# cgbur/llama2.zig

Hardware: AMD Instinct MI355X
Metric: tokens/s (argmax, -t 0) (higher is better)
Workload: dtype f32; 1 GPU; llama2-7b shape, fp32 llama2.c-v0 checkpoint (dim 4096, hidden 11008, L 32, H 32, kv 32, V 32000, S 2048), greedy from BOS, seeded synthetic weights; parallelism=1 GPU

## Files before the change

### llama2.zig_amd/csrc/forward.cpp

```cpp
#include <algorithm>
#include <cmath>
#include <cstdlib>
#include <cstring>
#include <mutex>

#include "batch_host.h"
#include "l2z_state.h"

namespace l2z {

struct Prof {
    std::vector<hipEvent_t> ev;
    std::vector<int> kind;
};

#define L2Z_LAUNCH(kind_id, expr)                                                         \
    do {                                                                                  \
        hipEvent_t _a = nullptr, _b = nullptr;                                            \
        if (prof) {                                                                       \
            L2Z_HIP(hipEventCreate(&_a));                                                 \
            L2Z_HIP(hipEventCreate(&_b));                                                 \
            L2Z_HIP(hipEventRecord(_a, st));                                              \
        }                                                                                 \
        L2Z_HIP(expr);                                                                    \
// ... 85 lines not shown
        L2Z_TRY(comm_allreduce(s->comm, s->part, s->x, dim, gi, was_pushed, st));
        if (prof != nullptr) {
            L2Z_HIP(hipEventRecord(eb, st));
            prof->ev.push_back(ea);
            prof->ev.push_back(eb);
            prof->kind.push_back(KIND_GATHER);
        }
        return L2Z_OK;
    };
    auto x_in = [&](MatvecArgs &a, const float *plain, int g, size_t count_per_rank) {
        a.x = plain;
        if (consume && g >= 1) a.xin = comm_ll_in(s->comm, g, count_per_rank);
    };
    auto push_to = [&](MatvecArgs &a, int which) {
        if (!can_push) return;
        a.push = s->d_push + which;
        a.push_ctl = ctl;
        a.push_gi = comm_gi(lc, gi + 1);
    };
    auto col_shard = [&](MatvecArgs &a, const float *wcols, const float *x_loc, int n_pad, int *epi) {
        a.w0 = wcols;
        a.x = x_loc;
        a.n = n_pad;
        a.rows0 = c.dim;
        a.out0 = s->part;
        a.resid = sh.rank == 0 ? s->x : nullptr;
        *epi = sh.rank == 0 ? EPI_RESID : EPI_STORE;
        push_to(a, 1);
    };
    const bool pk = s->packed_w && !sb && sh.world == 1 && !consume;
    const auto pk_slot = [&](int k, int l, int j = 0) -> const l2z_weights::PkMat * {
        return pk && ((s->packed_kinds >> k) & 1) ? w->pk_slot(k, l, j) : nullptr;
    };
    for (int l = 0; l < c.n_layers; l++) {
        float *kc = s->key_cache + (size_t)l * c.seq_len * sh.kvd_loc;
        float *vc = s->value_cache + (size_t)l * c.seq_len * sh.kvd_loc;
        const size_t kvh_stride = (size_t)c.seq_len * sh.hs;
        const bool fused = s->fused_qkv_attn && !split && only_stage < 0;
        if (fused && kind(KIND_QKV)) {
            FusedQkvAttnArgs a = {};
            a.wq = w->wq + (size_t)l * dim * dim;
            a.wk = w->wk + (size_t)l * dim * dim;
            a.wv = w->wv + (size_t)l * dim * dim;
            a.rms_w = w->rms_att + (size_t)l * dim; a.x = s->x; a.q_out = s->q;
            a.kcache = kc; a.vcache = vc; a.xb = s->xb; a.pos_ptr = s->d_pos; a.rope = s->rope;
            a.n = c.dim; a.head_size = sh.hs; a.seq_len = c.seq_len; a.kv_dim = sh.kvd_loc;
            a.kv_row = sh.hs; a.kv_head = kvh_stride;
            L2Z_LAUNCH(KIND_QKV, launch_fused_qkv_attn(a, c.n_heads, st));
        }
        if (!fused && want() && kind(KIND_QKV)) {
            MatvecArgs a = {};
            a.w0 = w->wq + (size_t)l * sh.dim_loc * dim;
            a.w1 = w->wk + (size_t)l * sh.kvd_loc * dim;
            a.w2 = w->wv + (size_t)l * sh.kvd_loc * dim;
            a.out0 = s->q; a.out1 = kc; a.out2 = vc;
            a.rows0 = sh.dim_loc; a.rows1 = sh.kvd_loc; a.rows2 = sh.kvd_loc;
            a.pos_stride1 = sh.hs; a.pos_stride2 = sh.hs; a.kv_head_stride = kvh_stride;
            a.n = c.dim; a.rms_w = w->rms_att + (size_t)l * dim;
            x_in(a, s->x, gi, sh.dim_loc);
            a.pos_ptr = s->d_pos; a.rope = s->rope; a.head_size = sh.hs; a.rope_segs = 2;
            const auto *pq = pk_slot(KIND_QKV, l, 0), *pkk = pk_slot(KIND_QKV, l, 1), *pv = pk_slot(KIND_QKV, l, 2);
            if (pq && pkk && pv) {
                a.pk = pq->p; a.pk_e = pq->e;
                a.pk1 = pkk->p; a.pk_e1 = pkk->e;
                a.pk2 = pv->p; a.pk_e2 = pv->e;
            }
// ... 15 lines not shown
                L2Z_LAUNCH(KIND_ATTN, launch_attention_split(a, sh.heads_loc, s->attn_nch,
                                                             s->d_attn_part, s->d_attn_cnt, st, variant == ATTN_SPLIT_S));
            else
                L2Z_LAUNCH(KIND_ATTN, launch_attention(a, sh.heads_loc, st, variant == ATTN_SHORT ? 1 : 0));
        }
        if (!sb) L2Z_TRY(gather(s->xb, sh.dim_loc));
        if (want() && kind(KIND_WO)) {
            MatvecArgs a = {};
            int epi = EPI_RESID;
            if (sb) {
                col_shard(a, w->wo + (size_t)l * dim * sh.dimc_pad, s->xb + sh.dim0, sh.dimc_pad, &epi);
            } else {
                a.w0 = w->wo + (size_t)l * sh.dim_loc * dim;
                a.out0 = s->x + sh.dim0; a.resid = s->x + sh.dim0;
                a.rows0 = sh.dim_loc; a.n = c.dim;
                x_in(a, s->xb, gi, sh.dim_loc);
                push_to(a, 1);
                if (const auto *p = pk_slot(KIND_WO, l)) { a.pk = p->p; a.pk_e = p->e; }
            }
            L2Z_LAUNCH(KIND_WO, launch_matvec(a, PRO_NONE, epi, mb, g_cus, st, nullptr, &pushed));
        }
        if (sb) L2Z_TRY(reduce());
        else L2Z_TRY(gather(s->x, sh.dim_loc));
        if (want() && kind(KIND_FFN13)) {
            MatvecArgs a = {};
            a.w0 = w->w1 + (size_t)l * sh.hid_loc * 2 * dim;
            a.w1 = w->w3 + (size_t)l * sh.hid_loc * 2 * dim;
            a.out0 = sb ? s->hb : s->hb + sh.hid0;
            a.rows0 = sh.hid_loc; a.rows1 = sh.hid_loc; a.n = c.dim;
            a.rms_w = w->rms_ffn + (size_t)l * dim;
            x_in(a, s->x, gi, sh.dim_loc);
            if (!sb) push_to(a, 2);
            if (const auto *p = pk_slot(KIND_FFN13, l)) { a.pk = p->p; a.pk_e = p->e; }
            L2Z_LAUNCH(KIND_FFN13, launch_matvec(a, PRO_RMS, EPI_SWIGLU, mb, g_cus, st, nullptr, &pushed));
        }
        if (!sb) L2Z_TRY(gather(s->hb, sh.hid_loc));
        if (want() && kind(KIND_FFN2)) {
            MatvecArgs a = {};
            int epi = EPI_RESID;
            if (sb) {
                col_shard(a, w->w2 + (size_t)l * dim * sh.hidc_pad, s->hb, sh.hidc_pad, &epi);
            } else {
                a.w0 = w->w2 + (size_t)l * sh.dim_loc * hid;
                a.out0 = s->x + sh.dim0; a.resid = s->x + sh.dim0;
                a.rows0 = sh.dim_loc; a.n = c.hidden_dim;
                x_in(a, s->hb, gi, sh.hid_loc);
                push_to(a, 1);
                if (const auto *p = pk_slot(KIND_FFN2, l)) { a.pk = p->p; a.pk_e = p->e; }
            }
            L2Z_LAUNCH(KIND_FFN2, launch_matvec(a, PRO_NONE, epi, mb, g_cus, st, nullptr, &pushed));
        }
        if (sb) L2Z_TRY(reduce());
        else L2Z_TRY(gather(s->x, sh.dim_loc));
    }
    if (want() && kind(KIND_CLS)) {
        MatvecArgs a = {};
        a.w0 = w->wcls; a.out0 = s->logits + sh.v0;
        a.rows0 = sh.v_loc; a.n = c.dim; a.rms_w = w->rms_final;
        x_in(a, s->x, gi, sh.dim_loc);
        a.part_val = s->d_part_val; a.part_idx = s->d_part_idx; a.row_offset = sh.v0;
        const bool fuse = (sh.world == 1 || xchg || (only_kind >= 0 && with_step && s->comm && !s->comm->nccl && !s->comm->p2p)) &&
                          matvec_vector_width(c.dim);
        int grid = 0;
        if (!xchg) push_to(a, 3);
        if (const auto *p = fuse ? pk_slot(KIND_CLS, 0) : nullptr) { a.pk = p->p; a.pk_e = p->e; }
        L2Z_LAUNCH(KIND_CLS, launch_matvec(a, PRO_RMS, fuse ? EPI_ARGMAX : EPI_STORE, mb, g_cus, st,
// ... 443 lines not shown
```

### llama2.zig_amd/csrc/l2z_internal.h

```cpp
#pragma once

#include <hip/hip_runtime.h>

#include <cstdarg>
#include <cstdint>
#include <cstdio>
#include <string>
#include <vector>

#include "../../include/llama2_hip.h"
#include "../../include/llama2_hip_test.h"

namespace l2z {

struct P2pArgs;

struct LLIn {
    const unsigned long long *slots;
    unsigned slot_floats;
    unsigned count;
    int gi;
    int *ctl;
    int *h_err;
    long long timeout_ticks;
// ... 61 lines not shown
    const float *tok_emb;
    float *x;
    int dim;
    int advance;
    int *epoch_ctl;
    int epoch_add;
    const P2pArgs *xchg;
    int xchg_gi;
};

struct MatvecArgs {
    const float *w0, *w1, *w2;
    float *out0, *out1, *out2;
    int rows0, rows1, rows2;
    int pos_stride1, pos_stride2;
    size_t kv_head_stride;
    int n;
    const float *x;
    const float *rms_w;
    const float *resid;
    const int *pos_ptr;
    const float2 *rope;
    int head_size;
    int rope_segs;
    float *part_val;
    int *part_idx;
    int row_offset;
    const P2pArgs *push;
    const int *push_ctl;
    int push_gi;
    LLIn xin;
    const uint32_t *pk, *pk1, *pk2;
    int pk_e, pk_e1, pk_e2;
    int tl_slot;
};

struct AttnArgs {
    const float *q;
    const float *kcache;
    const float *vcache;
    float *xb;
    const int *pos_ptr;
    int head_size;
    int kv_row;
    size_t kv_head;
    int kv_mul;
    int seq_len;
    const P2pArgs *push;
    const int *push_ctl;
    int push_gi;
    int tl_seq;
};


struct FusedQkvAttnArgs {
    const float *wq, *wk, *wv;
    const float *rms_w, *x;
    float *q_out;
    float *kcache, *vcache;
    float *xb;
    const int *pos_ptr;
    const float2 *rope;
    int n;
    int head_size, seq_len, kv_dim;
    int kv_row;
    size_t kv_head;
// ... 188 lines not shown
```

### llama2.zig_amd/csrc/l2z_state.h

```cpp
#pragma once
#include <cstdint>
#include <vector>

#include "kv_pages.h"
#include "l2z_comm.h"
#include "l2z_internal.h"
#include "tunables.h"

namespace l2z {

struct BatchScratch;
struct WideScratch;

struct Shard {
    int rank = 0, world = 1;
    int hs = 0;
    int dim0 = 0, dim_loc = 0;
    int kvd_loc = 0;
    int heads_loc = 0;
    int hid0 = 0, hid_loc = 0;
    int v0 = 0, v_loc = 0;
    bool scheme_b = false;
    int dimc_pad = 0, hidc_pad = 0;
};
int pad_cols(int n);
int make_shard(const l2z_config &c, const l2z_comm *comm, Shard *out);

enum ShardKind { REPL, BY_Q_HEADS, BY_KV_HEADS, BY_HIDDEN, BY_DIM_ROWS, BY_VOCAB, SKIP };

struct TensorDesc {
    const char *name;
    size_t offset;
    size_t layers, rows, cols;
    ShardKind kind;
    float scale, bias;
    size_t count() const { return layers * rows * cols; }
};
std::vector<TensorDesc> tensor_table(const l2z_config &c, bool shared);
void shard_rows(const TensorDesc &d, const Shard &s, size_t *r0, size_t *r1);
// ... 81 lines not shown
    void *sc_ws = nullptr, *sc_seq = nullptr;
    size_t sc_ws_bytes = 0;
    int sc_cap = 0, sc_slab_n = 0;
    int sc_slab_force = 0;
    float *d_probs = nullptr;
    float *h_stage = nullptr;
    float *d_smp_ctl = nullptr, *h_smp_ctl = nullptr, *d_smp_scratch = nullptr;
    float *d_part_val = nullptr;
    int *d_part_idx = nullptr;
    int n_part = 0;
    int n_part_step = 0, n_part_fwd = 0;
    float *d_attn_part = nullptr;
    int *d_attn_cnt = nullptr;
    int attn_nch = 0;
    int attn_split_pos = 0;
    int attn_short_pos = 0;
    int attn_split_wide_pos = 0;
    uint64_t graph_w_uid = 0;
    hipGraphExec_t g_forward[4] = {nullptr, nullptr, nullptr, nullptr}, g_step[4] = {nullptr, nullptr, nullptr, nullptr};
    hipGraphExec_t g_sample[4] = {nullptr, nullptr, nullptr, nullptr};
    bool use_graphs = true;
    int host_pos = 0;
    bool done = false;
    std::vector<int32_t> h_prompt;
    l2z::P2pArgs *d_push = nullptr;
    int n_gathers = 0;
    bool ll_consume = false;
    bool xchg_steps = false;
    bool logits_partial = false;
    bool fused_qkv_attn = false;
    int max_blocks = 0;
    bool packed_w = true;
    int packed_kinds = -1;
    int tl_attn_seq = 0;
    l2z::BatchScratch *bt = nullptr;
    float *rg_k = nullptr, *rg_v = nullptr;
    void *rg_tab = nullptr;
    int rg_cap = 0;
    l2z::WideScratch *wd = nullptr;
};

namespace l2z {

struct Prof;
int check_pair(const l2z_config *config, const l2z_runstate *s, const l2z_weights *w, bool paged_ok = false);
enum { ATTN_SHORT = 0, ATTN_HEAD = 1, ATTN_SPLIT_S = 2, ATTN_SPLIT = 3, ATTN_VARIANTS = 4 };
enum StepKind { STEP_NONE = 0, STEP_GREEDY = 1, STEP_SAMPLE = 2 };
int enqueue_forward(l2z_runstate *s, const l2z_weights *w, StepKind step, Prof *prof, int only_stage,
                    int variant, int only_kind = -1);
int attn_variant(const l2z_runstate *s, int pos);
int run_forward(l2z_runstate *s, const l2z_weights *w, StepKind step, int pos);
int ensure_logits(l2z_runstate *s);
void drop_graphs(l2z_runstate *s);

constexpr int kPrefillMinPrompt = L2Z_PREFILL_MIN_PROMPT;
bool prefill_enabled();
bool prefill_usable(const l2z_runstate *s);
bool prefill_shard_takes_the_unsharded_kernels(const l2z_config &c, const Shard &sh);
int prefill_check(const l2z_config *config, const l2z_runstate *s);
struct ScoreCall;
int prefill_tokens(l2z_runstate *s, const l2z_weights *w, const int32_t *tokens, int n_tokens, int pos0,
                   const ScoreCall *score = nullptr);

int prefill_scratch(l2z_runstate *s, int need);
int prefill_ragged_chunk(l2z_runstate *s, const l2z_weights *w, const int32_t *tokens, int P, const RaggedChunk &rg);
int prefill_last_logits(l2z_runstate *s, const l2z_weights *w);
// ... 19 lines not shown
```

### llama2.zig_amd/csrc/matvec.hip

```cpp
#include <type_traits>

#include "argmax_rule.h"
#include "matvec_device.h"
#include "packed_w.h"

namespace l2z {
namespace {

__device__ __forceinline__ void dot2_scalar(const float *__restrict__ pa,
                                            const float *__restrict__ pb, const float *xs, int n,
                                            float &ra, float &rb)
{
    const int lane = threadIdx.x & 63;
    float sa = 0.0f, sb = 0.0f;
    for (int j = lane; j < n; j += kWave) {
        const float xv = xs[j];
        sa = fmaf(pa[j], xv, sa);
        sb = fmaf(pb[j], xv, sb);
    }
    ra = wave_sum(sa);
    rb = wave_sum(sb);
}

template <int LPR>
struct MvGeom {
    static constexpr int RW = kWave / LPR;
    static constexpr int U = (LPR == 64) ? 4 : 6;
};

template <int LPR>
__device__ __forceinline__ void mv_load(const float *pa, const float *pb, int c0, int n4,
                                        v4f (&wa)[MvGeom<LPR>::U], v4f (&wb)[MvGeom<LPR>::U])
{
    constexpr int U = MvGeom<LPR>::U;
    const v4f *a4 = (const v4f *)pa, *b4 = (const v4f *)pb;
#pragma unroll
    for (int k = 0; k < U; k++) {
// ... 219 lines not shown
    {
        const bool last = b + 1 == n_batches;
        const uint32_t *src = pp + (last ? last_off : (size_t)b * (4 * 64 * pk::kMaxLaneDw) + (size_t)wave_u * (64 * pk::kMaxLaneDw));
        s_in[P] = (XC == 4 || !last) ? 4 : s_last;
        e31[P] = e_pt;
        pk_load_raw(src, threadIdx.x & 63, XC == 4 ? 4 : s_in[P], raw[P]);
    }
    template <int P>
    __device__ __forceinline__ void deliver()
    {
        if constexpr (XC == 4) {
            pk_decode_lane<4>(raw[P], e31[P], wa, wb);
        } else {
            switch (s_in[P]) {
                case 4: pk_decode_lane<4>(raw[P], e31[P], wa, wb); break;
                case 3: pk_decode_lane<3>(raw[P], e31[P], wa, wb); break;
                case 2: pk_decode_lane<2>(raw[P], e31[P], wa, wb); break;
                case 1: pk_decode_lane<1>(raw[P], e31[P], wa, wb); break;
                default: pk_decode_lane<0>(raw[P], e31[P], wa, wb); break;
            }
        }
    }
};

#ifdef L2Z_TIMELINE
constexpr int kMtlSlots = 256, kMtlBlocks = 512;
__device__ long long g_mtl[kMtlSlots * kMtlBlocks * 8];
unsigned long long g_mtl_launches = 0;
#define L2Z_MTL(i) tl[i] = wall_clock64()
#else
#define L2Z_MTL(i) do { } while (0)
#endif

template <int PRO, int EPI, int XC, bool LL, bool PK = false>
__global__ __launch_bounds__(kBlock) void matvec_row_kernel(const MatvecArgs a)
{
    constexpr int U = kRowU;
    using Src = typename std::conditional<PK, RowPacked<EPI, XC>, RowF32<EPI, XC>>::type;
    constexpr int NS = Src::kSets;
    extern __shared__ __attribute__((aligned(16))) float lds[];
#ifdef L2Z_TIMELINE
    long long tl[8] = {0, 0, 0, 0, 0, 0, 0, 0};
#endif
    L2Z_MTL(0);
    MvLocals m_ = mv_locals<EPI>(a);
    if constexpr (PK) m_.push = nullptr;
    const MvLocals m = m_;
    const int n4 = m.n >> 2;
    const int n_batches = (n4 + kBlock * U - 1) / (kBlock * U);
    const int n4_pad = n_batches * (kBlock * U);
    float *xs = lds;
    float *scratch = lds + 4 * n4_pad;
    float *part = scratch + kScratch;
    const v4f *xs4 = (const v4f *)xs;
    const int tid = threadIdx.x, lane = tid & 63, wave = tid >> 6;
    const int n_units = m.n_pairs;
    const int ustride = gridDim.x;

    XStage<PRO, XC, LL> xst;
    xst.issue(a.x, a.xin, a.rms_w, n4);
    int u = blockIdx.x;
    Src src;
    src.init(m, n4, n_batches);
    src.point(m, u);
    EpiIn ein = epi_prefetch<EPI>(m, u, tid == 0);
    EpiIn ein_next = ein;
    src.template issue<0>(0);
    L2Z_MTL(1);
    xst.finish(a.x, a.rms_w, m.n, n4_pad, xs, scratch);
    L2Z_MTL(2);

    int iu = u, ib = 0;
    bool imore = true;
    auto advance = [&]() __attribute__((always_inline)) {
        const MvStep s = mv_step(iu, ib, n_batches, ustride, n_units);
        imore = s.more;
        if (s.more) {
            if (s.unit_done) src.point(m, s.u_next);
            iu = s.u_next;
            ib = s.b_next;
        }
    };
    advance();

    v4f acc_a = {0.f, 0.f, 0.f, 0.f}, acc_b = {0.f, 0.f, 0.f, 0.f};
    ArgmaxCand best;
    int b = 0, parity = 0;
    auto step = [&](auto set, auto ahead) __attribute__((always_inline)) -> bool {
        constexpr int P = decltype(set)::value;
        const MvStep s = mv_step(u, b, n_batches, ustride, n_units);
        auto prefetch_next = [&]() __attribute__((always_inline)) {
            if (s.more && s.unit_done) ein_next = epi_prefetch<EPI>(m, s.u_next, tid == 0);
        };
        if constexpr (NS > 1) {
            prefetch_next();
            if constexpr (decltype(ahead)::value) {
                if constexpr (EPI == EPI_SWIGLU) asm volatile("s_waitcnt vmcnt(0)" ::: "memory");
                src.template issue<(P + 1) % NS>(ib);
                advance();
            }
        }
        src.template deliver<P>();
#pragma unroll
        for (int k = 0; k < U; k++) {
            const v4f xv = xs4[b * (kBlock * U) + tid + kBlock * k];
            acc_a = fma4(src.wa[k], xv, acc_a);
            acc_b = fma4(src.wb[k], xv, acc_b);
        }
        if constexpr (NS == 1) {
            prefetch_next();
            if (imore) {
                src.template issue<0>(ib);
                advance();
            }
        }
#ifdef L2Z_TIMELINE
        tl[6]++;
#endif
        if (s.unit_done) {
            const float sa = wave_sum(hsum4(acc_a));
            const float sb = wave_sum(hsum4(acc_b));
            float *pp_ = part + parity * (2 * kWaves);
            if (lane == 0) {
                pp_[wave] = sa;
                pp_[kWaves + wave] = sb;
            }
            __syncthreads();
            if (tid == 0) {
                const float ta = ((pp_[0] + pp_[1]) + pp_[2]) + pp_[3];
                const float tb = ((pp_[kWaves] + pp_[kWaves + 1]) + pp_[kWaves + 2]) + pp_[kWaves + 3];
                pair_epilogue<EPI>(m, u, ta, tb, true, ein);
                if (EPI == EPI_ARGMAX) {
                    const int ra_ = 2 * u, rb_ = ra_ + 1;
                    argmax_take(best, ta, ra_ + a.row_offset);
                    if (rb_ < m.total_rows) argmax_take(best, tb, rb_ + a.row_offset);
                }
            }
            ein = ein_next;
            parity ^= 1;
            acc_a = v4f{0.f, 0.f, 0.f, 0.f};
            acc_b = v4f{0.f, 0.f, 0.f, 0.f};
#ifdef L2Z_TIMELINE
            if (tl[7]++ == 0) L2Z_MTL(3);
            L2Z_MTL(4);
#endif
        }
        u = s.u_next;
        b = s.b_next;
        return !s.more;
    };
    using Set0 = std::integral_constant<int, 0>;
    using Set1 = std::integral_constant<int, 1>;
    static_assert(NS == 1 || NS == 2, "register sets of a source");
    if constexpr (NS == 1) {
        while (!step(Set0{}, std::false_type{})) {}
    } else {
        while (true) {
            if (!imore) { step(Set0{}, std::false_type{}); break; }
            step(Set0{}, std::true_type{});
            if (!imore) { step(Set1{}, std::false_type{}); break; }
            step(Set1{}, std::true_type{});
        }
    }
    if (EPI == EPI_ARGMAX && tid == 0) {
        a.part_val[blockIdx.x] = best.v;
        a.part_idx[blockIdx.x] = best.i;
    }
#ifdef L2Z_TIMELINE
    L2Z_MTL(5);
    if (tid == 0 && (unsigned)a.tl_slot < (unsigned)kMtlSlots && blockIdx.x < kMtlBlocks) {
        long long *o = g_mtl + ((size_t)a.tl_slot * kMtlBlocks + blockIdx.x) * 8;
        for (int i = 0; i < 8; i++) o[i] = tl[i];
    }
#endif
}

template <int PRO, int EPI>
__global__ __launch_bounds__(kBlock) void matvec_scalar_kernel(const MatvecArgs a)
{
    extern __shared__ __attribute__((aligned(16))) float lds[];
    const MvLocals m = mv_locals<EPI>(a);
    float *xs = lds;
    float *scratch = lds + ((m.n + 3) & ~3);
    stage_x_scalar<PRO>(a.x, a.rms_w, m.n, xs, scratch);
    const int lane = threadIdx.x & 63, wave = threadIdx.x >> 6;
    for (int u = blockIdx.x * kWaves + wave; u < m.n_pairs; u += gridDim.x * kWaves) {
        const float *pa, *pb;
        pair_rows<EPI>(m, u, pa, pb);
        float sa, sb;
        dot2_scalar(pa, pb, xs, m.n, sa, sb);
        pair_epilogue<EPI>(m, u, sa, sb, lane == 0, epi_prefetch<EPI>(m, u, lane == 0));
    }
}

int lpr_for(int n4)
{
    int l = 8;
    while (l < 64 && l * 6 < n4) l <<= 1;
    return l;
}

struct MvLaunch {
    const void *fn;
    int lpr, u;
};

template <int PRO, int EPI, int LPR, int XC, bool LL>
MvLaunch mv_entry()
{
    return {reinterpret_cast<const void *>(&matvec_kernel<PRO, EPI, LPR, XC, LL>), LPR, MvGeom<LPR>::U};
}

template <int PRO, int EPI, bool LL>
MvLaunch mv_pick(int lpr, bool big_x)
{
    if (lpr == 8) return mv_entry<PRO, EPI, 8, 4, LL>();
    if (lpr == 16) return mv_entry<PRO, EPI, 16, 4, LL>();
    if (lpr == 32) return mv_entry<PRO, EPI, 32, 4, LL>();
    return big_x ? mv_entry<PRO, EPI, 64, 12, LL>() : mv_entry<PRO, EPI, 64, 4, LL>();
}

template <int PRO, int EPI, bool LL, bool PK = false>
const void *mv_row_fn(bool big_x)
{
    return big_x ? reinterpret_cast<const void *>(&matvec_row_kernel<PRO, EPI, 12, LL, PK>)
                 : reinterpret_cast<const void *>(&matvec_row_kernel<PRO, EPI, 4, LL, PK>);
}

#define L2Z_MV_COMBOS(X)                     \
    X(PRO_NONE, EPI_STORE,  0, 1, 0)         \
    X(PRO_NONE, EPI_RESID,  1, 1, 1)         \
    X(PRO_RMS,  EPI_STORE,  1, 1, 0)         \
    X(PRO_RMS,  EPI_ROPE,   1, 1, 1)         \
    X(PRO_RMS,  EPI_SWIGLU, 1, 1, 1)         \
    X(PRO_RMS,  EPI_ARGMAX, 1, 0, 1)
#define L2Z_IF_1(...) __VA_ARGS__
#define L2Z_IF_0(...)

const void *mv_row_pick_packed(int pro, int epi, bool big_x)
{
#define X(P, E, LL, SC, PK) L2Z_IF_##PK(if (pro == P && epi == E) return mv_row_fn<P, E, false, true>(big_x);)
    L2Z_MV_COMBOS(X)
#undef X
    return nullptr;
}

const void *mv_row_pick(int pro, int epi, bool big_x, bool ll)
{
#define X(P, E, LL, SC, PK)                                           \
    if (pro == P && epi == E && !ll) return mv_row_fn<P, E, false>(big_x); \
    L2Z_IF_##LL(if (pro == P && epi == E && ll) return mv_row_fn<P, E, true>(big_x);)
    L2Z_MV_COMBOS(X)
#undef X
    return nullptr;
}

MvLaunch mv_pick_pe(int pro, int epi, int lpr, bool big_x, bool vec, bool ll)
{
#define X(P, E, LL, SC, PK)                                                                \
    if (pro == P && epi == E && vec && !ll) return mv_pick<P, E, false>(lpr, big_x);       \
    L2Z_IF_##LL(if (pro == P && epi == E && vec && ll) return mv_pick<P, E, true>(lpr, big_x);) \
    L2Z_IF_##SC(if (pro == P && epi == E && !vec && !ll)                                   \
                    return MvLaunch{reinterpret_cast<const void *>(&matvec_scalar_kernel<P, E>), 0, 0};)
    L2Z_MV_COMBOS(X)
#undef X
    return {nullptr, 0, 0};
}
#undef L2Z_MV_COMBOS
#undef L2Z_IF_1
#undef L2Z_IF_0

__global__ __launch_bounds__(256) void stream_read_kernel(const v4f *__restrict__ p, size_t n4, float *out)
{
    constexpr int U = 8;
    size_t i = (size_t)blockIdx.x * 256 * U + threadIdx.x;
    const size_t stride = (size_t)gridDim.x * 256 * U;
    v4f acc = {0.f, 0.f, 0.f, 0.f};
    for (; i + 256 * (U - 1) < n4; i += stride) {
        v4f r[U];
#pragma unroll
        for (int k = 0; k < U; k++) r[k] = ldg_nt(p + i + 256 * k);
#pragma unroll
        for (int k = 0; k < U; k++) acc += r[k];
    }
    const float s = (acc.x + acc.y) + (acc.z + acc.w);
    if (s == 123.456f) out[blockIdx.x] = s;
}

}

size_t matvec_lds_bytes(int n) { return (size_t)(4 * ((n >> 2) + 1024) + kScratch + 4 * kWaves + 4) * sizeof(float); }

// ... 6 lines not shown
    hipLaunchKernelGGL(stream_read_kernel, dim3(n_cus * 8), dim3(256), 0, st, (const v4f *)p, n_floats / 4, out);
    return hipGetLastError();
}

hipError_t launch_matvec(const MatvecArgs &a_in, int pro, int epi, int max_blocks_per_cu, int n_cus,
                         hipStream_t st, int *out_grid, bool *pushed)
{
    MatvecArgs a = a_in;
    if (max_blocks_per_cu > 8) max_blocks_per_cu = 8;
    bool vec = (a.n % 4) == 0 && aligned16(a.x) && aligned16(a.w0);
    if (a.rows1 > 0) vec = vec && aligned16(a.w1);
    if (a.rows2 > 0) vec = vec && aligned16(a.w2);
    if (pro == PRO_RMS) vec = vec && aligned16(a.rms_w);
    if (epi == EPI_SWIGLU && a.rows1 != a.rows0) return hipErrorInvalidValue;
    const int total_rows = a.rows0 + a.rows1 + a.rows2;
    const int n_pairs = (epi == EPI_SWIGLU) ? a.rows0 : (total_rows + 1) / 2;
    if (n_pairs <= 0 || a.n <= 0) return hipErrorInvalidValue;
    const int n4 = a.n >> 2;
    const int lpr = lpr_for(n4);
    if (epi == EPI_ARGMAX && (!vec || a.rows1 != 0 || a.rows2 != 0)) return hipErrorNotSupported;
    const Tunables &tn = tunables();
    const bool use_row = vec && n4 >= 1024 && (n4 % 64) == 0;
    const bool ll = a.xin.slots != nullptr;
    if (ll && !vec) return hipErrorNotSupported;
    if (a.pk != nullptr && (!use_row || ll || !pk::width_ok(a.n))) return hipErrorInvalidValue;
    if (a.pk != nullptr) a.push = nullptr;
    if (a.pk != nullptr && epi != EPI_SWIGLU &&
        ((a.rows1 > 0 && a.pk1 == nullptr) || (a.rows2 > 0 && a.pk2 == nullptr) || a.rows0 % 2 || a.rows1 % 2 || a.rows2 % 2))
        return hipErrorInvalidValue;
    MvLaunch k = {nullptr, 0, 0};
    size_t lds;
    int n_units;
    const auto padded = [n4](int batch) { return ((n4 + batch - 1) / batch) * batch; };
    if (use_row) {
        k.fn = a.pk != nullptr ? mv_row_pick_packed(pro, epi, a.n > 4096) : mv_row_pick(pro, epi, a.n > 4096, ll);
        lds = (size_t)(4 * padded(kBlock * kRowU) + kScratch + 4 * kWaves) * sizeof(float);
        n_units = n_pairs;
    } else if (vec) {
        k = mv_pick_pe(pro, epi, lpr, a.n > 4096, true, ll);
        if (k.fn == nullptr) return hipErrorInvalidValue;
        lds = (size_t)(4 * padded(k.lpr * k.u) + kScratch) * sizeof(float);
        const int rw = kWave / k.lpr;
        n_units = (n_pairs + rw - 1) / rw;
    } else {
        k = mv_pick_pe(pro, epi, lpr, a.n > 4096, false, ll);
        lds = (size_t)(((a.n + 3) & ~3) + kScratch) * sizeof(float);
        n_units = n_pairs;
    }
    if (k.fn == nullptr) return hipErrorInvalidValue;
    if (lds > 64 * 1024) {
        hipError_t e = hipFuncSetAttribute(k.fn, hipFuncAttributeMaxDynamicSharedMemorySize, (int)lds);
        if (e != hipSuccess) return e;
    }
    int occ = 0;
    if (hipOccupancyMaxActiveBlocksPerMultiprocessor(&occ, k.fn, kBlock, lds) != hipSuccess || occ < 1)
        occ = 1;
    if (occ > max_blocks_per_cu) occ = max_blocks_per_cu;
    if (use_row && occ > tn.row_blocks) occ = tn.row_blocks;
    int resident = occ * n_cus;
    if (tn.grid_cap > 0 && resident > tn.grid_cap) resident = tn.grid_cap;
    int grid;
    if (use_row) {
        grid = n_units;
        if (grid > resident) {
            const int per_block = (n_units + resident - 1) / resident;
            grid = (n_units + per_block - 1) / per_block;
        }
    } else {
        const int blocks_needed = (n_units + kWaves - 1) / kWaves;
        grid = blocks_needed;
        if (grid > resident) {
            const int per_wave = (n_units + resident * kWaves - 1) / (resident * kWaves);
            grid = (n_units + per_wave * kWaves - 1) / (per_wave * kWaves);
        }
    }
    if (out_grid) *out_grid = grid;
    if (!vec || epi == EPI_ROPE || a.rows2 != 0 || (epi != EPI_SWIGLU && a.rows1 != 0)) a.push = nullptr;
    if (pushed) *pushed = a.push != nullptr;
#ifdef L2Z_TIMELINE
    a.tl_slot = use_row ? (int)(g_mtl_launches++ % kMtlSlots) : -1;
#endif
    void *args[] = {&a};
    return hipLaunchKernel(k.fn, dim3(grid), dim3(kBlock), args, lds, st);
}

}

#ifdef L2Z_TIMELINE
extern "C" int l2z_matvec_timeline_dump(long long *out, unsigned long long *n_launches)
{
    if (hipDeviceSynchronize() != hipSuccess) return 1;
    if (hipMemcpyFromSymbol(out, HIP_SYMBOL(l2z::g_mtl), sizeof(long long) * l2z::kMtlSlots * l2z::kMtlBlocks * 8) != hipSuccess) return 1;
    *n_launches = l2z::g_mtl_launches;
    return 0;
}
// ... 2 lines not shown
```

### llama2.zig_amd/csrc/runstate.cpp

```cpp
#include <algorithm>
#include <cmath>
#include <cstdlib>
#include <cstring>
#include <mutex>
#include <vector>

#include "l2z_state.h"

using namespace l2z;

static int runstate_make(const l2z_config *config, const l2z_comm *comm, l2z_kvpool *pool, l2z_runstate **out)
{
    L2Z_CHECK(config != nullptr && out != nullptr, L2Z_ERR_INVALID, "runstate_init: null argument");
    const int dev = current_device_for(comm);
    L2Z_TRY(ensure_device(dev));
    Shard sh;
    L2Z_TRY(make_shard(*config, comm, &sh));
    const l2z_config &c = *config;
    const size_t att_lds = attention_lds_bytes(sh.hs, c.seq_len, sh.hs % 4 == 0 && sh.kvd_loc % 4 == 0);
    L2Z_CHECK(att_lds <= 160 * 1024, L2Z_ERR_INVALID,
              "seq_len %d needs %zu bytes of LDS for attention scores (max 163840)", c.seq_len,
              att_lds);
    const int n_max = c.dim > c.hidden_dim ? c.dim : c.hidden_dim;
    L2Z_CHECK(matvec_lds_bytes(n_max) <= 160 * 1024, L2Z_ERR_INVALID,
// ... 25 lines not shown
        }
    }

    const size_t kv = (size_t)c.n_layers * c.seq_len * sh.kvd_loc;
    hipError_t e = hipStreamCreateWithFlags(&s->stream, hipStreamNonBlocking);
    auto alloc = [&](void **p, size_t bytes) {
        if (e == hipSuccess) e = hipMalloc(p, bytes ? bytes : 4);
        if (e == hipSuccess) e = hipMemset(*p, 0, bytes ? bytes : 4);
    };
    alloc((void **)&s->x, (size_t)c.dim * 4);
    alloc((void **)&s->xb, ((size_t)c.dim + 256) * 4);
    alloc((void **)&s->hb, ((size_t)c.hidden_dim + 256) * 4);
    if (sh.scheme_b) alloc((void **)&s->part, (size_t)c.dim * 4);
    alloc((void **)&s->q, (size_t)c.dim * 4);
    alloc((void **)&s->logits, (size_t)c.vocab_size * 4);
    if (pool == nullptr) {
        alloc((void **)&s->key_cache, kv * 4);
        alloc((void **)&s->value_cache, kv * 4);
    } else {
        s->pg.init(c.seq_len);
        alloc((void **)&s->d_pages, s->pg.pages.size() * 4);
        if (e == hipSuccess) e = hipHostMalloc((void **)&s->h_pages, s->pg.pages.size() * 4, hipHostMallocDefault);
        s->pages_dirty = true;
    }
    alloc((void **)&s->rope, (size_t)c.seq_len * (sh.hs / 2) * sizeof(float2));
    alloc((void **)&s->d_token, 4);
    alloc((void **)&s->d_pos, 4);
    alloc((void **)&s->d_n_prompt, 4);
    alloc((void **)&s->d_argmax, 4);
    alloc((void **)&s->d_prompt, (size_t)c.seq_len * 4);
    alloc((void **)&s->d_out_tokens, (size_t)c.seq_len * 4);
    alloc((void **)&s->d_part_val, (size_t)matvec_max_grid(g_cus) * 4);
    alloc((void **)&s->d_part_idx, (size_t)matvec_max_grid(g_cus) * 4);
    {
        const int mode = tn.attn_split;
        int nch = mode > 0 ? mode : attention_split_chunks(c.n_heads, g_cus);
        if (nch > 16) nch = 16;
        s->attn_split_pos = mode > 0 ? 0 : 256;
        if (tn.attn_split_pos >= 0) s->attn_split_pos = tn.attn_split_pos;
        if (mode == 0 || c.seq_len <= s->attn_split_pos) nch = 0;
        s->attn_split_wide_pos = attention_split_wide_pos(c.seq_len);
        s->attn_short_pos = attention_short_pos(sh.hs, c.seq_len);
        if (nch > 1 && s->attn_short_pos > s->attn_split_pos) s->attn_short_pos = s->attn_split_pos;
        if (nch > 1) {
            s->attn_nch = nch;
            alloc((void **)&s->d_attn_part, attention_split_part_floats(sh.heads_loc, sh.hs, nch) * 4);
            alloc((void **)&s->d_attn_cnt, (size_t)sh.heads_loc * 4);
        }
    }
    if (comm_uses_p2p(comm) && e == hipSuccess) {
        AttnArgs aa = {};
        aa.q = s->q; aa.kcache = s->key_cache; aa.vcache = s->value_cache;
        aa.head_size = sh.hs; aa.kv_row = sh.hs; aa.kv_head = (size_t)c.seq_len * sh.hs;
        const bool want_consume = tn.p2p_consume >= 0 ? tn.p2p_consume != 0 : (sh.world <= 2 || c.dim < 4096);
        s->ll_consume = !sh.scheme_b && want_consume && matvec_vector_width(c.dim) &&
                        matvec_vector_width(c.hidden_dim) && attention_push_supported(aa);
        P2pArgs t[4];
        comm_p2p_args(comm, s->xb, (size_t)sh.dim_loc, s->ll_consume, &t[0]);
        comm_p2p_args(comm, sh.scheme_b ? s->part : s->x, sh.scheme_b ? (size_t)c.dim : (size_t)sh.dim_loc, s->ll_consume, &t[1]);
        comm_p2p_args(comm, s->hb, (size_t)sh.hid_loc, s->ll_consume, &t[2]);
        comm_p2p_args(comm, s->logits, (size_t)sh.v_loc, false, &t[3]);
        alloc((void **)&s->d_push, sizeof t);
        if (e == hipSuccess) e = hipMemcpy(s->d_push, t, sizeof t, hipMemcpyHostToDevice);
        s->xchg_steps = tn.argmax_xchg != 0 && matvec_vector_width(c.dim) && sh.v_loc >= 2 && comm->slot_floats >= 2 * (size_t)sh.world;
    }
    if (e != hipSuccess) {
// ... 24 lines not shown
        pool->live++;
    }
    *out = s;
    return L2Z_OK;
}

extern "C" int l2z_runstate_init(const l2z_config *config, const l2z_comm *comm, l2z_runstate **out)
{
    return runstate_make(config, comm, nullptr, out);
}

extern "C" int l2z_runstate_init_paged(const l2z_config *config, l2z_kvpool *pool, l2z_runstate **out)
{
    L2Z_CHECK(config != nullptr && pool != nullptr && out != nullptr, L2Z_ERR_INVALID, "l2z_runstate_init_paged: null argument");
    L2Z_CHECK(memcmp(config, &pool->cfg, sizeof *config) == 0, L2Z_ERR_INVALID,
              "l2z_runstate_init_paged: the pool was made with another config");
    L2Z_CHECK(current_device_for(nullptr) == pool->device, L2Z_ERR_INVALID,
              "l2z_runstate_init_paged: the pool lives on device %d, the current device is another", pool->device);
    return runstate_make(config, nullptr, pool, out);
}

extern "C" void l2z_runstate_free(l2z_runstate *s)
{
    if (!s) return;
    (void)hipSetDevice(s->device);
    if (s->stream) (void)hipStreamSynchronize(s->stream);
    for (int v = 0; v < l2z::ATTN_VARIANTS; v++) {
        if (s->g_forward[v]) (void)hipGraphExecDestroy(s->g_forward[v]);
        if (s->g_step[v]) (void)hipGraphExecDestroy(s->g_step[v]);
        if (s->g_sample[v]) (void)hipGraphExecDestroy(s->g_sample[v]);
    }
    void *ptrs[] = {s->x, s->xb, s->hb, s->q, s->logits, s->key_cache, s->value_cache, s->rope,
                    s->d_token, s->d_pos, s->d_prompt, s->d_n_prompt, s->d_out_tokens, s->d_argmax,
                    s->d_probs, s->d_part_val, s->d_part_idx, s->d_attn_part, s->d_attn_cnt, s->pf_x, s->pf_xn, s->pf_q,
                    s->pf_att, s->pf_h1, s->pf_stage, s->pf_part, s->pf_tokens, s->d_push, s->pf_sk.part, s->pf_sk.cnt, s->pf_sk.x3, s->pf_sk.x3b, s->part, s->sc_ws, s->sc_seq,
                    s->rg_k, s->rg_v, s->rg_tab, s->d_smp_ctl, s->d_smp_scratch};
    for (void *p : ptrs)
        if (p) (void)hipFree(p);
    if (s->h_stage) (void)hipHostFree(s->h_stage);
    if (s->h_smp_ctl) (void)hipHostFree(s->h_smp_ctl);
    if (s->pool == nullptr) {
        if (s->d_pages) (void)hipFree(s->d_pages);
        if (s->h_pages) (void)hipHostFree(s->h_pages);
    }
    l2z::kv_runstate_free(s);
    l2z::batch_free(s);
    l2z::wide_free(s);
    if (s->stream) (void)hipStreamDestroy(s->stream);
    delete s;
}

extern "C" int l2z_runstate_form(const l2z_runstate *s, int *form)
{
    L2Z_CHECK(s != nullptr && form != nullptr, L2Z_ERR_INVALID, "l2z_runstate_form: bad arguments");
    *form = s->sh.scheme_b ? 8 : 0;
    return L2Z_OK;
}

extern "C" int l2z_runstate_read(l2z_runstate *s, const char *name, size_t offset, size_t count,
                                 float *out)
{
    L2Z_CHECK(s && name && out, L2Z_ERR_INVALID, "l2z_runstate_read: null argument");
    const l2z_config &c = s->cfg;
    const size_t kv = (size_t)c.n_layers * c.seq_len * s->sh.kvd_loc;
    const float *p = nullptr;
    size_t n = 0;
    const std::string k = name;
// ... 134 lines not shown
```

### llama2.zig_amd/csrc/tunables.cpp

```cpp
#include "tunables.h"

#include <cstdlib>
#include <cstring>

namespace l2z {
namespace {

void env_int(const char *name, int *v)
{
    if (const char *e = getenv(name))
        if (*e) *v = atoi(e);
}

Tunables read_env()
{
    Tunables t;
    env_int("L2Z_GRID_CAP", &t.grid_cap);
    env_int("L2Z_ATTN_SPLIT", &t.attn_split);
    env_int("L2Z_ATTN_SPLIT_POS", &t.attn_split_pos);
    env_int("L2Z_FUSE_SMALL", &t.fuse_small);
    env_int("L2Z_SCHEME_B", &t.scheme_b);
    env_int("L2Z_NO_GRAPH", &t.no_graph);
    if (const char *e = getenv("L2Z_COMM")) t.prefer_rccl = strcmp(e, "rccl") == 0;
    env_int("L2Z_ARGMAX_XCHG", &t.argmax_xchg);
    env_int("L2Z_P2P_CONSUME", &t.p2p_consume);
    if (const char *e = getenv("L2Z_P2P_TIMEOUT_S"))
        if (*e) t.p2p_timeout_s = atoll(e);
    env_int("L2Z_P2P_BULK_MB", &t.p2p_bulk_mb);
    env_int("L2Z_PREFILL", &t.prefill);
    env_int("L2Z_PF_CHUNK", &t.pf_chunk);
    env_int("L2Z_PF_PANEL", &t.pf_panel);
    env_int("L2Z_PF_PANEL_MAX", &t.pf_panel_max);
    env_int("L2Z_PF_X3", &t.pf_x3);
    env_int("L2Z_PF_X3_STREAM_MIN", &t.pf_x3_stream_min);
    env_int("L2Z_PF_FUSE_PLANES", &t.pf_fuse_planes);
    env_int("L2Z_PACKED_W", &t.packed_w);
    env_int("L2Z_PACKED_KINDS", &t.packed_kinds);
    return t;
}

}

namespace {
Tunables &mutable_tunables()
{
    static Tunables t = read_env();
    return t;
}
}

const Tunables &tunables() { return mutable_tunables(); }

int prefill_chunk_tokens()
{
    int n = tunables().pf_chunk > 0 ? tunables().pf_chunk : 1024;
    if (n < 16) n = 16;
    if (n > 2048) n = 2048;
    return n;
}

int prefill_next_chunk(int remaining)
{
    if (tunables().pf_chunk > 0) return remaining < prefill_chunk_tokens() ? remaining : prefill_chunk_tokens();
    return remaining >= 1024 ? 1024 : remaining < 512 ? remaining : 512;
}

bool tunables_set(const char *name, long long v)
{
    Tunables &t = mutable_tunables();
    struct { const char *n; int *p; } ints[] = {
        {"L2Z_GRID_CAP", &t.grid_cap}, {"L2Z_ATTN_SPLIT", &t.attn_split}, {"L2Z_ATTN_SPLIT_POS", &t.attn_split_pos},
        {"L2Z_FUSE_SMALL", &t.fuse_small}, {"L2Z_NO_GRAPH", &t.no_graph}, {"L2Z_SCHEME_B", &t.scheme_b},
        {"L2Z_COMM_RCCL", &t.prefer_rccl}, {"L2Z_ARGMAX_XCHG", &t.argmax_xchg}, {"L2Z_P2P_CONSUME", &t.p2p_consume},
        {"L2Z_P2P_BULK_MB", &t.p2p_bulk_mb}, {"L2Z_PREFILL", &t.prefill}, {"L2Z_PF_CHUNK", &t.pf_chunk},
        {"L2Z_PF_PANEL", &t.pf_panel}, {"L2Z_PF_PANEL_MAX", &t.pf_panel_max},
        {"L2Z_PF_X3", &t.pf_x3}, {"L2Z_PF_X3_STREAM_MIN", &t.pf_x3_stream_min},
        {"L2Z_PF_FUSE_PLANES", &t.pf_fuse_planes}, {"L2Z_PACKED_W", &t.packed_w},
        {"L2Z_PACKED_KINDS", &t.packed_kinds}};
    for (auto &e : ints)
        if (strcmp(e.n, name) == 0) {
            *e.p = (int)v;
            return true;
        }
    if (strcmp(name, "L2Z_P2P_TIMEOUT_S") == 0) {
        t.p2p_timeout_s = v;
        return true;
    }
    return false;
}

}
```

### llama2.zig_amd/csrc/tunables.h

```cpp
#pragma once

namespace l2z {

struct Tunables {
    int grid_cap = 0;
    int attn_split = -1;
    int attn_split_pos = -1;
    int fuse_small = 1;
    int no_graph = 0;
    int prefer_rccl = 0;
    int p2p_consume = -1;
    int argmax_xchg = 1;
    long long p2p_timeout_s = 20;
    int scheme_b = 0;
    int p2p_bulk_mb = -1;
    int prefill = 1;
    int pf_chunk = 0;
    int pf_panel = 1;
    int pf_x3 = 1;
    int pf_x3_stream_min = 33;
    int pf_fuse_planes = 1;
    int packed_w = 1;
    int packed_kinds = -1;
    int pf_panel_max = -1;

    static constexpr int row_blocks = 2;
    static constexpr int max_blocks_per_cu = 8;
    static constexpr int p2p_push = 1;
    static constexpr int reduce_block = 128;
    static constexpr int pf_skinny_max = 64;
};

const Tunables &tunables();
int prefill_chunk_tokens();
int prefill_next_chunk(int remaining);
bool tunables_set(const char *env_name, long long value);

}
```

Measured before the change: 241.4 tokens/s.

## Add dynamic row dealing with atomic work-stealing heads to FFN13 matvec

Adds a hybrid static/dynamic scheduler to the packed row matvec used for the FFN w1/w3 SwiGLU projection. Each block first processes about 7/8 of its fair share of row units statically. It then draws the remaining units from one of 16 atomic counters, grouped by block, through a 4-entry LDS lookahead ring. The aim is to reduce tail imbalance across CUs, at the cost of atomic traffic, a per-layer counter buffer that must be reset by the last drawer, and extra control flow in the inner loop. A timeline-only register read is also added.

```diff
diff --git a/llama2.zig_amd/csrc/forward.cpp b/llama2.zig_amd/csrc/forward.cpp
--- a/llama2.zig_amd/csrc/forward.cpp
+++ b/llama2.zig_amd/csrc/forward.cpp
@@ -141,6 +141,9 @@
     const auto pk_slot = [&](int k, int l, int j = 0) -> const l2z_weights::PkMat * {
         return pk && ((s->packed_kinds >> k) & 1) ? w->pk_slot(k, l, j) : nullptr;
     };
+    const auto deal_slot = [&](int j) -> unsigned * {
+        return s->d_row_deal != nullptr && !sb && sh.world == 1 ? s->d_row_deal + (size_t)j * row_deal::kSlotWords : nullptr;
+    };
     for (int l = 0; l < c.n_layers; l++) {
         float *kc = s->key_cache + (size_t)l * c.seq_len * sh.kvd_loc;
         float *vc = s->value_cache + (size_t)l * c.seq_len * sh.kvd_loc;
@@ -222,6 +225,7 @@
             x_in(a, s->x, gi, sh.dim_loc);
             if (!sb) push_to(a, 2);
             if (const auto *p = pk_slot(KIND_FFN13, l)) { a.pk = p->p; a.pk_e = p->e; }
+            a.deal_heads = deal_slot(l);
             L2Z_LAUNCH(KIND_FFN13, launch_matvec(a, PRO_RMS, EPI_SWIGLU, mb, g_cus, st, nullptr, &pushed));
         }
         if (!sb) L2Z_TRY(gather(s->hb, sh.hid_loc));
diff --git a/llama2.zig_amd/csrc/l2z_internal.h b/llama2.zig_amd/csrc/l2z_internal.h
--- a/llama2.zig_amd/csrc/l2z_internal.h
+++ b/llama2.zig_amd/csrc/l2z_internal.h
@@ -117,6 +117,7 @@
     LLIn xin;
     const uint32_t *pk, *pk1, *pk2;
     int pk_e, pk_e1, pk_e2;
+    unsigned *deal_heads;
     int tl_slot;
 };
 
diff --git a/llama2.zig_amd/csrc/l2z_state.h b/llama2.zig_amd/csrc/l2z_state.h
--- a/llama2.zig_amd/csrc/l2z_state.h
+++ b/llama2.zig_amd/csrc/l2z_state.h
@@ -5,6 +5,7 @@
 #include "kv_pages.h"
 #include "l2z_comm.h"
 #include "l2z_internal.h"
+#include "row_deal.h"
 #include "tunables.h"
 
 namespace l2z {
@@ -152,6 +153,7 @@
     int max_blocks = 0;
     bool packed_w = true;
     int packed_kinds = -1;
+    unsigned *d_row_deal = nullptr;
     int tl_attn_seq = 0;
     l2z::BatchScratch *bt = nullptr;
     float *rg_k = nullptr, *rg_v = nullptr;
diff --git a/llama2.zig_amd/csrc/matvec.hip b/llama2.zig_amd/csrc/matvec.hip
--- a/llama2.zig_amd/csrc/matvec.hip
+++ b/llama2.zig_amd/csrc/matvec.hip
@@ -3,6 +3,7 @@
 #include "argmax_rule.h"
 #include "matvec_device.h"
 #include "packed_w.h"
+#include "row_deal.h"
 
 namespace l2z {
 namespace {
@@ -288,7 +289,7 @@
 #define L2Z_MTL(i) do { } while (0)
 #endif
 
-template <int PRO, int EPI, int XC, bool LL, bool PK = false>
+template <int PRO, int EPI, int XC, bool LL, bool PK = false, bool DEAL = false>
 __global__ __launch_bounds__(kBlock) void matvec_row_kernel(const MatvecArgs a)
 {
     constexpr int U = kRowU;
@@ -300,7 +301,7 @@
 #endif
     L2Z_MTL(0);
     MvLocals m_ = mv_locals<EPI>(a);
-    if constexpr (PK) m_.push = nullptr;
+    if constexpr (PK || DEAL) m_.push = nullptr;
     const MvLocals m = m_;
     const int n4 = m.n >> 2;
     const int n_batches = (n4 + kBlock * U - 1) / (kBlock * U);
@@ -312,6 +313,30 @@
     const int tid = threadIdx.x, lane = tid & 63, wave = tid >> 6;
     const int n_units = m.n_pairs;
     const int ustride = gridDim.x;
+    int *ring = (int *)(part + 4 * kWaves);
+    row_deal::Plan dp = {};
+    row_deal::Head dh = {};
+    unsigned *dhead = nullptr;
+    if constexpr (DEAL) {
+        dp = row_deal::row_deal_plan(n_units, gridDim.x, row_deal::kHeads);
+        dh = row_deal::head_for(dp, blockIdx.x);
+        dhead = a.deal_heads + dh.h * row_deal::kHeadStride;
+    }
+    static_assert(row_deal::kAhead == 4, "the ring is indexed with & 3");
+    auto row_step = [&](int uu, int bb, int jj) __attribute__((always_inline)) -> MvStep {
+        if constexpr (!DEAL) {
+            return mv_step(uu, bb, n_batches, ustride, n_units);
+        } else {
+            MvStep s;
+            s.unit_done = (bb + 1 == n_batches);
+            s.b_next = s.unit_done ? 0 : bb + 1;
+            s.u_next = uu;
+            if (s.unit_done)
+                s.u_next = jj + 1 < dp.static_rounds ? uu + ustride : __builtin_amdgcn_readfirstlane(ring[(jj + 1) & 3]);
+            s.more = s.u_next >= 0;
+            return s;
+        }
+    };
 
     XStage<PRO, XC, LL> xst;
     xst.issue(a.x, a.xin, a.rms_w, n4);
@@ -326,13 +351,16 @@
     xst.finish(a.x, a.rms_w, m.n, n4_pad, xs, scratch);
     L2Z_MTL(2);
 
-    int iu = u, ib = 0;
+    int iu = u, ib = 0, ij = 0;
     bool imore = true;
     auto advance = [&]() __attribute__((always_inline)) {
-        const MvStep s = mv_step(iu, ib, n_batches, ustride, n_units);
+        const MvStep s = row_step(iu, ib, ij);
         imore = s.more;
         if (s.more) {
-            if (s.unit_done) src.point(m, s.u_next);
+            if (s.unit_done) {
+                src.point(m, s.u_next);
+                ij++;
+            }
             iu = s.u_next;
             ib = s.b_next;
         }
@@ -341,10 +369,12 @@
 
     v4f acc_a = {0.f, 0.f, 0.f, 0.f}, acc_b = {0.f, 0.f, 0.f, 0.f};
     ArgmaxCand best;
-    int b = 0, parity = 0;
+    int b = 0, parity = 0, uj = 0;
+    unsigned ticket = 0;
+    bool ticket_out = false, drawing = true;
     auto step = [&](auto set, auto ahead) __attribute__((always_inline)) -> bool {
         constexpr int P = decltype(set)::value;
-        const MvStep s = mv_step(u, b, n_batches, ustride, n_units);
+        const MvStep s = row_step(u, b, uj);
         auto prefetch_next = [&]() __attribute__((always_inline)) {
             if (s.more && s.unit_done) ein_next = epi_prefetch<EPI>(m, s.u_next, tid == 0);
         };
@@ -357,6 +387,21 @@
             }
         }
         src.template deliver<P>();
+        if constexpr (DEAL) {
+            if (b == 0 && tid == 0) {
+                if (ticket_out) {
+                    const int got = row_deal::unit_of(dp, dh, ticket);
+                    ring[(uj + 3) & 3] = got;
+                    if (row_deal::last_draw(dh, ticket)) __hip_atomic_store(dhead, 0u, __ATOMIC_RELAXED, __HIP_MEMORY_SCOPE_AGENT);
+                    drawing = got >= 0;
+                    ticket_out = false;
+                }
+                if (drawing && uj + row_deal::kAhead >= dp.static_rounds) {
+                    ticket = __hip_atomic_fetch_add(dhead, 1u, __ATOMIC_RELAXED, __HIP_MEMORY_SCOPE_AGENT);
+                    ticket_out = true;
+                }
+            }
+        }
 #pragma unroll
         for (int k = 0; k < U; k++) {
             const v4f xv = xs4[b * (kBlock * U) + tid + kBlock * k];
@@ -392,6 +437,7 @@
                     if (rb_ < m.total_rows) argmax_take(best, tb, rb_ + a.row_offset);
                 }
             }
+            if constexpr (DEAL) uj++;
             ein = ein_next;
             parity ^= 1;
             acc_a = v4f{0.f, 0.f, 0.f, 0.f};
@@ -424,6 +470,8 @@
     }
 #ifdef L2Z_TIMELINE
     L2Z_MTL(5);
+    tl[7] |= ((long long)(__builtin_amdgcn_s_getreg(20 | (3 << 11)) & 15) << 32) |
+             ((long long)(__builtin_amdgcn_s_getreg(4 | (15 << 11)) & 0xffff) << 40);
     if (tid == 0 && (unsigned)a.tl_slot < (unsigned)kMtlSlots && blockIdx.x < kMtlBlocks) {
         long long *o = g_mtl + ((size_t)a.tl_slot * kMtlBlocks + blockIdx.x) * 8;
         for (int i = 0; i < 8; i++) o[i] = tl[i];
@@ -476,34 +524,42 @@
     return big_x ? mv_entry<PRO, EPI, 64, 12, LL>() : mv_entry<PRO, EPI, 64, 4, LL>();
 }
 
-template <int PRO, int EPI, bool LL, bool PK = false>
+template <int PRO, int EPI, bool LL, bool PK = false, bool DEAL = false>
 const void *mv_row_fn(bool big_x)
 {
-    return big_x ? reinterpret_cast<const void *>(&matvec_row_kernel<PRO, EPI, 12, LL, PK>)
-                 : reinterpret_cast<const void *>(&matvec_row_kernel<PRO, EPI, 4, LL, PK>);
-}
-
-#define L2Z_MV_COMBOS(X)                     \
-    X(PRO_NONE, EPI_STORE,  0, 1, 0)         \
-    X(PRO_NONE, EPI_RESID,  1, 1, 1)         \
-    X(PRO_RMS,  EPI_STORE,  1, 1, 0)         \
-    X(PRO_RMS,  EPI_ROPE,   1, 1, 1)         \
-    X(PRO_RMS,  EPI_SWIGLU, 1, 1, 1)         \
-    X(PRO_RMS,  EPI_ARGMAX, 1, 0, 1)
+    return big_x ? reinterpret_cast<const void *>(&matvec_row_kernel<PRO, EPI, 12, LL, PK, DEAL>)
+                 : reinterpret_cast<const void *>(&matvec_row_kernel<PRO, EPI, 4, LL, PK, DEAL>);
+}
+
+#define L2Z_MV_COMBOS(X)                        \
+    X(PRO_NONE, EPI_STORE,  0, 1, 0, 0)         \
+    X(PRO_NONE, EPI_RESID,  1, 1, 1, 0)         \
+    X(PRO_RMS,  EPI_STORE,  1, 1, 0, 0)         \
+    X(PRO_RMS,  EPI_ROPE,   1, 1, 1, 0)         \
+    X(PRO_RMS,  EPI_SWIGLU, 1, 1, 1, 1)         \
+    X(PRO_RMS,  EPI_ARGMAX, 1, 0, 1, 0)
 #define L2Z_IF_1(...) __VA_ARGS__
 #define L2Z_IF_0(...)
 
 const void *mv_row_pick_packed(int pro, int epi, bool big_x)
 {
-#define X(P, E, LL, SC, PK) L2Z_IF_##PK(if (pro == P && epi == E) return mv_row_fn<P, E, false, true>(big_x);)
+#define X(P, E, LL, SC, PK, DL) L2Z_IF_##PK(if (pro == P && epi == E) return mv_row_fn<P, E, false, true>(big_x);)
     L2Z_MV_COMBOS(X)
 #undef X
     return nullptr;
 }
 
+const void *mv_row_pick_dealt(int pro, int epi, bool big_x)
+{
+#define X(P, E, LL, SC, PK, DL) L2Z_IF_##DL(if (pro == P && epi == E) return mv_row_fn<P, E, false, true, true>(big_x);)
+    L2Z_MV_COMBOS(X)
+#undef X
+    return nullptr;
+}
+
 const void *mv_row_pick(int pro, int epi, bool big_x, bool ll)
 {
-#define X(P, E, LL, SC, PK)                                           \
+#define X(P, E, LL, SC, PK, DL)                                       \
     if (pro == P && epi == E && !ll) return mv_row_fn<P, E, false>(big_x); \
     L2Z_IF_##LL(if (pro == P && epi == E && ll) return mv_row_fn<P, E, true>(big_x);)
     L2Z_MV_COMBOS(X)
@@ -513,7 +569,7 @@
 
 MvLaunch mv_pick_pe(int pro, int epi, int lpr, bool big_x, bool vec, bool ll)
 {
-#define X(P, E, LL, SC, PK)                                                                \
+#define X(P, E, LL, SC, PK, DL)                                                            \
     if (pro == P && epi == E && vec && !ll) return mv_pick<P, E, false>(lpr, big_x);       \
     L2Z_IF_##LL(if (pro == P && epi == E && vec && ll) return mv_pick<P, E, true>(lpr, big_x);) \
     L2Z_IF_##SC(if (pro == P && epi == E && !vec && !ll)                                   \
@@ -586,8 +642,10 @@
     size_t lds;
     int n_units;
     const auto padded = [n4](int batch) { return ((n4 + batch - 1) / batch) * batch; };
+    const void *dealt_fn = nullptr;
     if (use_row) {
         k.fn = a.pk != nullptr ? mv_row_pick_packed(pro, epi, a.n > 4096) : mv_row_pick(pro, epi, a.n > 4096, ll);
+        if (a.deal_heads != nullptr && a.pk != nullptr) dealt_fn = mv_row_pick_dealt(pro, epi, a.n > 4096);
         lds = (size_t)(4 * padded(kBlock * kRowU) + kScratch + 4 * kWaves) * sizeof(float);
         n_units = n_pairs;
     } else if (vec) {
@@ -614,7 +672,16 @@
     int resident = occ * n_cus;
     if (tn.grid_cap > 0 && resident > tn.grid_cap) resident = tn.grid_cap;
     int grid;
-    if (use_row) {
+    if (dealt_fn != nullptr && row_deal::row_deal_plan(n_units, row_deal::dealt_grid(n_units, resident), row_deal::kHeads).pool > 0) {
+        k.fn = dealt_fn;
+        grid = row_deal::dealt_grid(n_units, resident);
+        lds += row_deal::kAhead * sizeof(int);
+        if (lds > 64 * 1024) {
+            hipError_t e = hipFuncSetAttribute(k.fn, hipFuncAttributeMaxDynamicSharedMemorySize, (int)lds);
+            if (e != hipSuccess) return e;
+        }
+    } else if (use_row) {
+        a.deal_heads = nullptr;
         grid = n_units;
         if (grid > resident) {
             const int per_block = (n_units + resident - 1) / resident;
diff --git a/llama2.zig_amd/csrc/row_deal.h b/llama2.zig_amd/csrc/row_deal.h
--- /dev/null
+++ b/llama2.zig_amd/csrc/row_deal.h
@@ -0,0 +1,89 @@
+#pragma once
+
+#if defined(__HIPCC__)
+#define L2Z_RD_FN __host__ __device__ inline
+#else
+#define L2Z_RD_FN inline
+#endif
+
+namespace l2z {
+namespace row_deal {
+
+constexpr int kHeads = 16;
+constexpr int kGroup = 8;
+constexpr int kHeadStride = 32;
+constexpr int kSlotWords = kHeads * kHeadStride;
+constexpr int kAhead = 4;
+constexpr int kStaticNum = 7, kStaticDen = 8;
+
+struct Plan {
+    int n_units, grid;
+    int heads;
+    int static_rounds;
+    int pool_base;
+    int pool;
+};
+
+L2Z_RD_FN int dealt_grid(int n_units, int resident)
+{
+    if (resident < 1) resident = 1;
+    return n_units < resident ? (n_units < 1 ? 1 : n_units) : resident;
+}
+
+L2Z_RD_FN Plan row_deal_plan(int n_units, int grid, int n_heads)
+{
+    Plan p;
+    if (n_units < 0) n_units = 0;
+    if (grid < 1) grid = 1;
+    p.n_units = n_units;
+    p.grid = grid;
+    const int share = n_units / grid;
+    if (n_heads < 1 || share <= kAhead) {
+        p.heads = 0;
+        p.static_rounds = (n_units + grid - 1) / grid;
+        p.pool_base = n_units;
+        p.pool = 0;
+        return p;
+    }
+    int rounds = (int)((long long)share * kStaticNum / kStaticDen);
+    if (rounds < kAhead) rounds = kAhead;
+    const int groups = (grid + kGroup - 1) / kGroup;
+    p.heads = n_heads < groups ? n_heads : groups;
+    p.static_rounds = rounds;
+    p.pool_base = rounds * grid;
+    p.pool = n_units - p.pool_base;
+    return p;
+}
+
+L2Z_RD_FN int static_unit(const Plan &p, int block, int k) { return block + k * p.grid; }
+L2Z_RD_FN int head_of(const Plan &p, int block) { return (block / kGroup) % p.heads; }
+L2Z_RD_FN int pool_of(const Plan &p, int h) { return (p.pool - h + p.heads - 1) / p.heads; }
+L2Z_RD_FN int blocks_of(const Plan &p, int h)
+{
+    const int round = kGroup * p.heads;
+    int rest = p.grid % round - h * kGroup;
+    rest = rest < 0 ? 0 : (rest > kGroup ? kGroup : rest);
+    return p.grid / round * kGroup + rest;
+}
+L2Z_RD_FN int draws_of(const Plan &p, int h) { return pool_of(p, h) + blocks_of(p, h); }
+
+struct Head {
+    int h;
+    unsigned pool, draws;
+};
+L2Z_RD_FN Head head_for(const Plan &p, int block)
+{
+    Head hd;
+    hd.h = head_of(p, block);
+    hd.pool = (unsigned)pool_of(p, hd.h);
+    hd.draws = (unsigned)draws_of(p, hd.h);
+    return hd;
+}
+L2Z_RD_FN int unit_of(const Plan &p, const Head &hd, unsigned ticket)
+{
+    return ticket < hd.pool ? p.pool_base + (int)ticket * p.heads + hd.h : -1;
+}
+L2Z_RD_FN bool last_draw(const Head &hd, unsigned ticket) { return ticket + 1 == hd.draws; }
+
+}
+}
diff --git a/llama2.zig_amd/csrc/runstate.cpp b/llama2.zig_amd/csrc/runstate.cpp
--- a/llama2.zig_amd/csrc/runstate.cpp
+++ b/llama2.zig_amd/csrc/runstate.cpp
@@ -81,6 +81,8 @@
     alloc((void **)&s->d_out_tokens, (size_t)c.seq_len * 4);
     alloc((void **)&s->d_part_val, (size_t)matvec_max_grid(g_cus) * 4);
     alloc((void **)&s->d_part_idx, (size_t)matvec_max_grid(g_cus) * 4);
+    if (tn.row_deal != 0 && sh.world == 1)
+        alloc((void **)&s->d_row_deal, (size_t)c.n_layers * row_deal::kSlotWords * sizeof(unsigned));
     {
         const int mode = tn.attn_split;
         int nch = mode > 0 ? mode : attention_split_chunks(c.n_heads, g_cus);
@@ -171,7 +173,7 @@
     }
     void *ptrs[] = {s->x, s->xb, s->hb, s->q, s->logits, s->key_cache, s->value_cache, s->rope,
                     s->d_token, s->d_pos, s->d_prompt, s->d_n_prompt, s->d_out_tokens, s->d_argmax,
-                    s->d_probs, s->d_part_val, s->d_part_idx, s->d_attn_part, s->d_attn_cnt, s->pf_x, s->pf_xn, s->pf_q,
+                    s->d_probs, s->d_part_val, s->d_part_idx, s->d_attn_part, s->d_attn_cnt, s->d_row_deal, s->pf_x, s->pf_xn, s->pf_q,
                     s->pf_att, s->pf_h1, s->pf_stage, s->pf_part, s->pf_tokens, s->d_push, s->pf_sk.part, s->pf_sk.cnt, s->pf_sk.x3, s->pf_sk.x3b, s->part, s->sc_ws, s->sc_seq,
                     s->rg_k, s->rg_v, s->rg_tab, s->d_smp_ctl, s->d_smp_scratch};
     for (void *p : ptrs)
diff --git a/llama2.zig_amd/csrc/tunables.cpp b/llama2.zig_amd/csrc/tunables.cpp
--- a/llama2.zig_amd/csrc/tunables.cpp
+++ b/llama2.zig_amd/csrc/tunables.cpp
@@ -36,6 +36,7 @@
     env_int("L2Z_PF_FUSE_PLANES", &t.pf_fuse_planes);
     env_int("L2Z_PACKED_W", &t.packed_w);
     env_int("L2Z_PACKED_KINDS", &t.packed_kinds);
+    env_int("L2Z_ROW_DEAL", &t.row_deal);
     return t;
 }
 
@@ -76,7 +77,7 @@
         {"L2Z_PF_PANEL", &t.pf_panel}, {"L2Z_PF_PANEL_MAX", &t.pf_panel_max},
         {"L2Z_PF_X3", &t.pf_x3}, {"L2Z_PF_X3_STREAM_MIN", &t.pf_x3_stream_min},
         {"L2Z_PF_FUSE_PLANES", &t.pf_fuse_planes}, {"L2Z_PACKED_W", &t.packed_w},
-        {"L2Z_PACKED_KINDS", &t.packed_kinds}};
+        {"L2Z_PACKED_KINDS", &t.packed_kinds}, {"L2Z_ROW_DEAL", &t.row_deal}};
     for (auto &e : ints)
         if (strcmp(e.n, name) == 0) {
             *e.p = (int)v;
diff --git a/llama2.zig_amd/csrc/tunables.h b/llama2.zig_amd/csrc/tunables.h
--- a/llama2.zig_amd/csrc/tunables.h
+++ b/llama2.zig_amd/csrc/tunables.h
@@ -22,6 +22,7 @@
     int pf_fuse_planes = 1;
     int packed_w = 1;
     int packed_kinds = -1;
+    int row_deal = 1;
     int pf_panel_max = -1;
 
     static constexpr int row_blocks = 2;
```

Result: no change. 242.9 tokens/s, median of 3 (+0.6%).
